# jweyn/DLWP-CS

Measured on AMD Instinct MI355X. Metric: cubed-sphere samples/sec (fwd+bwd), higher is better.
Workload: dtype bf16; 1 GPU; unet2 C48: x (32,6,48,48,14) per GPU, 14 out channels, base 32, MSE + Adam, fwd+bwd+update, bf16 activations + bf16 MFMA, fp32 master weights / gradients / Adam; global_batch=32, parallelism=dp1, hip_graphs=True

## Files before the change

dlwp-cs_amd/csrc/wgrad_batch.hip:

```cpp
#include <stdio.h>
#include <stdlib.h>
#include <string.h>
#include <vector>
#include "common.h"
#include "mfma_common.h"

namespace dlwpcs {
static const int g_wb_tags[] = {prof_register_tag("wgrad_batch_kernel"), prof_register_tag("wb_reduce_kernel"),
                                prof_register_tag("wb_reduce_kernel(apply)")};


constexpr int WB_MAX_LAYERS = DLWPCS_WGRAD_BATCH_MAX;
constexpr uint32_t WB_MAGIC = 0x57424c31u;

enum {
    WB_V_3_8_22 = 0,
    WB_V_3_8_21,
    WB_V_3_8_12,
    WB_V_3_8_11,
    WB_V_3_2_8,
    WB_V_3_2_16,
    WB_V_1_8_11,
    WB_V_1_8_D2,
    WB_V_F32_3,
    WB_V_F32_1,
    WB_V_F32_3_X2,
    WB_V_F32_3_H2,
    WB_V_F32_1_D2,
    WB_NVARIANTS
};

struct WbLayer {
    int32_t B, Nin, No, C0, C1, Cin, Cout, up0;
    int32_t halo, KS, W2, tile_rows_max, pix, nbands, pix_cap, variant;
    uint32_t magicW2, magicNo, magicN, magicB, magicNb;
    int32_t CT, NT, ncit, ncot, cin_logical, flip, want_bias, group_base, has_np, slot_floats, mask;
    float alpha, vmax;
    int32_t pad0, pad1;
};
static_assert(sizeof(WbLayer) == 144, "WbLayer layout");

struct WbSeg {
    int32_t layer, cls, cit, cot, t_first, t_last;
    uint32_t slot_off;
    int32_t bias;
};

struct WbGroup { uint32_t off, stride; int32_t count, pad; };

struct WbHeader {
    uint32_t magic, n_layers, n_segments, n_workers, n_groups, lds_bytes;
    uint32_t off_layers, off_segs, off_groups, total_bytes;
    uint64_t ws_floats;
    uint32_t red_first[WB_MAX_LAYERS + 1];
    uint32_t seg_start[257];
};

struct WbPtrs {
    const void *src0[WB_MAX_LAYERS], *src1[WB_MAX_LAYERS], *dz[WB_MAX_LAYERS], *y[WB_MAX_LAYERS];
    const int32_t *table[WB_MAX_LAYERS];
};
struct WbAdam {
    float *p, *g, *m, *v;
    const int32_t *state;
    const float *hyper;
    int32_t on;
    int32_t apply_only;
};
struct WbRedLayer { int32_t KS, Cin, Cout, want_bias, TC, TN, ncot, group_base, flip; };
struct WbRedPack { bf16_t *wf, *wb; float *bp; int32_t CGf, NTf, CGb, NTb, f32; };
struct WbPackArgs { WbRedPack l[WB_MAX_LAYERS]; };
struct WbRedPtrs {
    float *dw_eq[WB_MAX_LAYERS], *dw_pol[WB_MAX_LAYERS], *dw_np[WB_MAX_LAYERS];
    float *db_eq[WB_MAX_LAYERS], *db_pol[WB_MAX_LAYERS], *db_np[WB_MAX_LAYERS];
    uint32_t first[WB_MAX_LAYERS + 1];
    uint32_t live;
    uint32_t adam;
    uint32_t n_layers, off_groups;
    WbRedLayer lay[WB_MAX_LAYERS];
};

#ifndef DLWPCS_WB_SCHED
#define DLWPCS_WB_SCHED 1
#endif
template <int N> __device__ __forceinline__ void wb_sched_pairs() {
    if constexpr (N > 0) {
        __builtin_amdgcn_sched_group_barrier(0x008, 1, 0);
        __builtin_amdgcn_sched_group_barrier(0x100, 2, 0);
        wb_sched_pairs<N - 1>();
    }
}
#if DLWPCS_WB_SCHED == 1
#define WB_SCHED() do {                                                                   \
        __builtin_amdgcn_sched_group_barrier(0x100, 2, 0);       \
        wb_sched_pairs<TAPS>();                                                           \
    } while (0)
#else
#define WB_SCHED() do {                                                                   \
        __builtin_amdgcn_sched_group_barrier(0x100, 2 * TAPS + 2, 0);                     \
        __builtin_amdgcn_sched_group_barrier(0x008, TAPS, 0);                             \
    } while (0)
#endif

template <typename T> __device__ __forceinline__ T load_uniform(const T &g) {
    T out;
    const int *s = reinterpret_cast<const int *>(&g);
    int *d = reinterpret_cast<int *>(&out);
#pragma unroll
    for (int i = 0; i < (int)(sizeof(T) / 4); ++i) d[i] = __builtin_amdgcn_readfirstlane(s[i]);
    return out;
}

#define WB_SEG_ATTR __attribute__((noinline))
#ifndef DLWPCS_WB_PRODUCER_PRIO
#define DLWPCS_WB_PRODUCER_PRIO 0
#endif
#ifdef DLWPCS_WB_TL
constexpr int TL_WORKERS = 256, TL_MAX = 8;
#define WB_TL_DECL(kind_) \
    const bool tl_on = dbg != nullptr && (threadIdx.x & 255) == 0; \
    long long *tl_base = dbg + ((size_t)blockIdx.x * 2 + (kind_)) * TL_MAX; \
    long long tl_a[TL_MAX] = {0, 0, 0, 0, 0, 0, 0, 0}; \
    long long tl_prev = (long long)__builtin_amdgcn_s_memtime();
#define WB_TL(bucket_) do { const long long t_ = (long long)__builtin_amdgcn_s_memtime(); tl_a[bucket_] += t_ - tl_prev; tl_prev = t_; } while (0)
#define WB_TL_END() do { if (tl_on) { _Pragma("unroll") for (int q_ = 0; q_ < TL_MAX; ++q_) tl_base[q_] += tl_a[q_]; } } while (0)
#else
#define WB_TL_DECL(kind_)
#define WB_TL(tag_)
#define WB_TL_END()
#endif
template <int KS, int XV, int QX, int CT, int NT, int DV, bool MASK = false>
__device__ WB_SEG_ATTR void wb_segment(const WbLayer &Lg, const WbSeg &sgg, const void *src0, const void *src1,
                                           const void *dzp, const void *yp, const int32_t *table, float *ws, char *smem,
                                           long long *dbg) {
    const WbLayer L = load_uniform(Lg);
    const WbSeg sg = load_uniform(sgg);
    constexpr int QD = DV == 8 ? 4 : 8;
    constexpr int QDT = QD * NT;
    typedef typename VecT<bf16_t, DV>::type DVec;
    typedef typename VecT<bf16_t, XV>::type XVec;
    constexpr int TAPS = KS * KS;
    constexpr int PB = 64;
    constexpr int NCT = 256;
    constexpr int QXT = QX * CT;
    constexpr int IT_X = XV == 8 ? (CT == 2 ? 10 : 8) : 16;
    constexpr int CAP_PIX = (CT == 2 || NT == 2) ? 192 : 384;
    constexpr int IT_DY = CAP_PIX * QDT / NCT;
    constexpr int NPH = 4 / (CT * NT);
    constexpr int RSLOTS = TAPS - TAPS / NPH;
    constexpr int RED_FLOATS = 4 * RSLOTS * 1024;
    static_assert(CT * NT * NPH == 4, "four consumer waves");
    static_assert(CT == 1 || (XV == 8 && QX == 4), "two ci tiles per worker need full 16-B X vectors");
    static_assert(NCT % QXT == 0 && NCT % QDT == 0, "thread -> channel-vector maps must not depend on the item");

    const int pix_cap = L.pix_cap;
    constexpr int XCAP_PIX = (IT_X / CT) * NCT / QX;
    constexpr int plane_bytes = XCAP_PIX * PB;
    constexpr int x_bytes = CT * plane_bytes;
    constexpr int dzplane_bytes = CAP_PIX * PB;
    constexpr int buf_bytes = x_bytes + NT * dzplane_bytes;

    const int nfaces = sg.cls == 0 ? 4 : 1, fbase = sg.cls == 0 ? 0 : (sg.cls == 1 ? 4 : 5);
    const int n_my = sg.t_last - sg.t_first;
    const int face_pix = L.No * L.No;
    const int tid = threadIdx.x;
    (void)nfaces;

    struct Item { int b, f, combo, m0, npix, y0, nitems; };
    auto item_of = [&](int k) {
        Item it;
        const int t = sg.t_first + max(min(k, n_my - 1), 0);
        it.combo = L.magicB ? __umulhi((uint32_t)t, L.magicB) : t;
        it.b = t - it.combo * L.B;
        const int fl = L.magicNb ? __umulhi((uint32_t)it.combo, L.magicNb) : it.combo;
        const int band = it.combo - fl * L.nbands;
        it.f = fbase + fl;
        it.m0 = band * L.pix;
        it.npix = min(L.pix, face_pix - it.m0);
        it.y0 = __umulhi((uint32_t)it.m0, L.magicNo);
        const int ylast = __umulhi((uint32_t)(it.m0 + it.npix - 1), L.magicNo);
        it.nitems = (ylast - it.y0 + KS) * L.W2 * QXT;
        return it;
    };
    ws = reinterpret_cast<float *>(((uint64_t)(uint32_t)__builtin_amdgcn_readfirstlane((int)((uint64_t)ws >> 32)) << 32) |
                                   (uint32_t)__builtin_amdgcn_readfirstlane((int)(uint32_t)(uint64_t)ws));
    float *slot = ws + sg.slot_off;

    if (tid >= NCT) {
        const int ptid = tid - NCT;
        if (DLWPCS_WB_PRODUCER_PRIO) __builtin_amdgcn_s_setprio(DLWPCS_WB_PRODUCER_PRIO);
        WB_TL_DECL(0)
        const int qd = ptid % QDT;
        const int g0 = L.up0 ? (L.Nin >> 1) : L.Nin;
        const int M = L.Nin + KS - 1;
        const int co = sg.cot * 32 * NT + (qd / QD) * 32 + (qd % QD) * DV;
        const bool co_ok = co < L.Cout;
        const bool want_bias = sg.bias != 0;
        const uint32_t mthr1 = (uint32_t)L.pad0;
        float bsum[DV];
#pragma unroll
        for (int u = 0; u < DV; ++u) bsum[u] = 0.f;
        auto uni_ptr = [](const void *q) {
            return reinterpret_cast<const char *>(((uint64_t)(uint32_t)__builtin_amdgcn_readfirstlane((int)((uint64_t)q >> 32)) << 32) |
                                                  (uint32_t)__builtin_amdgcn_readfirstlane((int)(uint32_t)(uint64_t)q));
        };
        const char *const x0_u = uni_ptr(src0), *const x1_u = uni_ptr(src1);
        const char *const dz_u = uni_ptr(dzp), *const y_u = uni_ptr(yp);
        const int32_t *const table_u = reinterpret_cast<const int32_t *>(uni_ptr(table));
        const uint32_t s0_bytes = (uint32_t)((size_t)6 * g0 * g0 * L.C0 * 2), s1_bytes = (uint32_t)((size_t)6 * L.Nin * L.Nin * L.C1 * 2);
        constexpr int ITP = IT_X / CT;
        static_assert(IT_X % CT == 0 && NCT % QX == 0, "plane-major load map");
        const int qx = ptid % QX;
        struct Plane { int cs, stride; bool all0, up, ok, f0; };
        bool straddle = false;
        auto mkplane = [&](int pl) {
            Plane q;
            const int c_lo = sg.cit * 32 * CT + pl * 32, c_hi = min(c_lo + 32, L.Cin);
            const int cxp = c_lo + qx * XV;
            q.all0 = c_hi <= L.C0;
            straddle |= c_lo < L.C0 && c_hi > L.C0;
            q.ok = cxp < L.Cin;
            q.f0 = cxp < L.C0;
            q.cs = q.f0 ? cxp : cxp - L.C0;
            q.stride = q.f0 ? L.C0 : L.C1;
            q.up = q.f0 && L.up0;
            return q;
        };
        const Plane P0 = mkplane(0), P1 = mkplane(CT - 1);
        auto nit_plane = [&](const Item &it) { return it.nitems / CT; };
        uint32_t xoff[IT_X];
        int cur_combo = -1;
        const rsrc_t rt = make_rsrc(table_u, L.halo ? (uint32_t)(6 * M * M * 4) : 0u);
        auto rebuild = [&](const Item &it) {
            const int nitp = nit_plane(it);
            int tbl[ITP];
#pragma unroll
            for (int j = 0; j < ITP; ++j) {
                const int e = min(ptid + j * NCT, nitp - 1);
                const int pix = e / QX;
                const int ty = __umulhi((uint32_t)pix, L.magicW2);
                const int tx = pix - ty * L.W2;
                tbl[j] = (int)__builtin_amdgcn_raw_buffer_load_b32(rt, (uint32_t)(((it.f * M + it.y0 + ty) * M + tx) * 4), 0, 0);
            }
#pragma unroll
            for (int j = 0; j < ITP; ++j) {
                const int e = min(ptid + j * NCT, nitp - 1);
                const int pix = e / QX;
                const int ty = __umulhi((uint32_t)pix, L.magicW2);
                const int tx = pix - ty * L.W2;
                const int iy = it.y0 + ty;
                const int ii = L.halo ? tbl[j] : (it.f * L.Nin + iy) * L.Nin + tx;
                const int r = __umulhi((uint32_t)ii, L.magicN);
                const int pix_up = (r >> 1) * g0 + ((ii - r * L.Nin) >> 1);
                {
                    const int spix = P0.up ? pix_up : ii;
// ... 14 lines not shown
            DVec dv[IT_DY], yv[MASK ? IT_DY : 1];
        };
        auto bld = [](rsrc_t r, uint32_t off, auto &dst) __attribute__((always_inline)) {
            typedef std::remove_reference_t<decltype(dst)> V;
#ifdef DLWPCS_WB_ABL_P
            if (DLWPCS_WB_ABL_P & 2) { memset(&dst, 0, sizeof(V)); asm volatile("" : "+v"(*reinterpret_cast<uint32_t *>(&dst))); return; }
#endif
            if constexpr (sizeof(V) == 16) {
                const u32x4 q = __builtin_amdgcn_raw_buffer_load_b128(r, off, 0, 0);
                dst = make_uint4(q.x, q.y, q.z, q.w);
            } else {
                dst = __builtin_amdgcn_raw_buffer_load_b32(r, off, 0, 0);
            }
        };
        auto issue = [&](const Item &it, Stage &st, bool live) {
            if (live && it.combo != cur_combo) rebuild(it);
            const rsrc_t r0 = make_rsrc(x0_u + (size_t)it.b * s0_bytes, live ? s0_bytes : 0u);
            const rsrc_t r1 = make_rsrc(x1_u ? x1_u + (size_t)it.b * s1_bytes : nullptr, live ? s1_bytes : 0u);
            if (!straddle) {
                const rsrc_t rp0 = make_rsrc(P0.all0 ? x0_u + (size_t)it.b * s0_bytes : (x1_u ? x1_u + (size_t)it.b * s1_bytes : nullptr),
                                             live ? (P0.all0 ? s0_bytes : s1_bytes) : 0u);
                const rsrc_t rp1 = make_rsrc(P1.all0 ? x0_u + (size_t)it.b * s0_bytes : (x1_u ? x1_u + (size_t)it.b * s1_bytes : nullptr),
                                             live ? (P1.all0 ? s0_bytes : s1_bytes) : 0u);
#pragma unroll
                for (int i = 0; i < IT_X; ++i) {
                    if (i % CT == 0) bld(rp0, xoff[i], st.xv[i]);
                    else bld(rp1, xoff[i], st.xv[i]);
                }
            } else {
#pragma unroll
                for (int i = 0; i < IT_X; ++i) {
                    XVec a, b;
                    const bool f0 = i % CT == 0 ? P0.f0 : P1.f0;
                    bld(r0, f0 ? xoff[i] : 0xffffffffu, a);
                    bld(r1, f0 ? 0xffffffffu : xoff[i], b);
                    st.xv[i] = a | b;
                }
            }
            const size_t rowbase = (((size_t)it.b * 6 + it.f) * face_pix + it.m0) * L.Cout * 2;
            const uint32_t dbytes = live ? (uint32_t)(it.npix * L.Cout * 2) : 0u;
            const rsrc_t rd = make_rsrc(dz_u + rowbase, dbytes);
#pragma unroll
            for (int i = 0; i < IT_DY; ++i) bld(rd, doff[i], st.dv[i]);
            if constexpr (MASK) {
                const rsrc_t ry = make_rsrc(y_u + rowbase, dbytes);
#pragma unroll
                for (int i = 0; i < IT_DY; ++i) bld(ry, doff[i], st.yv[i]);
            }
        };
        auto commit = [&](const Item &it, int k, Stage &st) {
            char *buf = smem + (k & 1) * buf_bytes;
            WB_TL(0);
#ifdef DLWPCS_WB_TL
            asm volatile("s_waitcnt vmcnt(%0)" :: "n"(IT_X + IT_DY + (MASK ? IT_DY : 0)) : "memory");
            WB_TL(1);
#endif
            char *const xbase = buf + (ptid / QX) * PB + qx * (XV * 2);
#pragma unroll
            for (int i = 0; i < IT_X; ++i) {
#ifdef DLWPCS_WB_ABL_P
                if (DLWPCS_WB_ABL_P & 1) { asm volatile("" :: "v"(*reinterpret_cast<uint32_t *>(&st.xv[i]))); continue; }
#endif
                *reinterpret_cast<XVec *>(xbase + (i % CT) * plane_bytes + (i / CT) * (NCT / QX) * PB) = st.xv[i];
            }
            char *const dbase = buf + x_bytes + (qd / QD) * dzplane_bytes + (ptid / QDT) * PB + (qd % QD) * (DV * 2);
#pragma unroll
            for (int i = 0; i < IT_DY; ++i) {
                if constexpr (MASK) {
                    if constexpr (DV == 8) vmask_pk(st.dv[i], st.yv[i], L.alpha, mthr1);
                    else vmask(st.dv[i], st.yv[i], L.alpha, L.vmax);
                }
                const DVec v = st.dv[i];
#ifdef DLWPCS_WB_ABL_P
                if (DLWPCS_WB_ABL_P & 1) { asm volatile("" :: "v"(*reinterpret_cast<const uint32_t *>(&v))); }
                else
#endif
                *reinterpret_cast<DVec *>(dbase + i * (NCT / QDT) * PB) = v;
#ifdef DLWPCS_WB_ABL_P
                if (DLWPCS_WB_ABL_P & 4) continue;
#endif
                if (want_bias) {
                    if constexpr (DV == 8) {
                        bsum[0] += bf_lo(v.x); bsum[1] += bf_hi(v.x); bsum[2] += bf_lo(v.y); bsum[3] += bf_hi(v.y);
                        bsum[4] += bf_lo(v.z); bsum[5] += bf_hi(v.z); bsum[6] += bf_lo(v.w); bsum[7] += bf_hi(v.w);
                    } else {
                        bsum[0] += bf_lo(v); bsum[1] += bf_hi(v);
                    }
                }
            }
            asm volatile("s_waitcnt lgkmcnt(0)" ::: "memory");
            WB_TL(2);
            __builtin_amdgcn_s_barrier();
            WB_TL(3);
        };
        {
            Stage A, B;
            Item i0 = item_of(0), i1 = item_of(1);
            issue(i0, A, true);
            issue(i1, B, 1 < n_my);
            const int npair = n_my >> 1;
            for (int pr = 0; pr < npair; ++pr) {
                const int k = 2 * pr;
                commit(i0, k, A);
                i0 = item_of(k + 2);
                issue(i0, A, k + 2 < n_my);
                commit(i1, k + 1, B);
                i1 = item_of(k + 3);
                issue(i1, B, k + 3 < n_my);
            }
            if (n_my & 1) commit(i0, n_my - 1, A);
        }
        __syncthreads();
        float *red = reinterpret_cast<float *>(smem) + RED_FLOATS;
        if (want_bias) {
#pragma unroll
            for (int u = 0; u < DV; ++u) red[ptid * DV + u] = bsum[u];
        }
        __syncthreads();
        if (want_bias && ptid < 32 * NT) {
            float sum = 0.f;
            const int cc = ptid & 31, pl = ptid >> 5;
            if (cc < QD * DV) {
                const int q = pl * QD + cc / DV;
#pragma unroll 4
                for (int ph = 0; ph < NCT / QDT; ++ph) sum += red[(ph * QDT + q) * DV + (cc % DV)];
            }
            slot[TAPS * (32 * CT) * (32 * NT) + ptid] = sum;
        }
        __syncthreads();
        WB_TL(4);
        WB_TL_END();
        return;
    }

    const int lane = tid & 63, wave = tid >> 6;
    const int half = lane >> 5, l31 = lane & 31;
    const int li = lane & 15;
    WB_TL_DECL(1)
    const int choff = ((((lane >> 4) & 1) * 16) + (li & 3) * 4) * 2;
    const int prow = li >> 2;
    f32x16 acc[TAPS];
#pragma unroll
    for (int t = 0; t < TAPS; ++t)
#pragma unroll
        for (int r = 0; r < 16; ++r) acc[t][r] = 0.f;
    const int nslab = pix_cap / 16;
    const int S = (((nslab + NPH - 1) / NPH) + 1) & ~1;
    const int wave_u = __builtin_amdgcn_readfirstlane(wave);
    const int ct = wave_u % CT, nt = (wave_u / CT) % NT, ph = wave_u / (CT * NT);
    constexpr int DSTEP = 16 * NPH;
    const int stq = (int)__umulhi((uint32_t)DSTEP, L.magicNo), str = DSTEP - stq * L.No;
    const int stepA = (stq * L.W2 + str) * PB, wrapA = (L.W2 - L.No) * PB, rowB = L.W2 * PB;
    const int mlane = 16 * ph + 8 * half + prow;
    for (int k = 0; k < n_my; ++k) {
        WB_TL(1);
        __syncthreads();
        WB_TL(0);
        const int buf0 = (k & 1) * buf_bytes;
        const Item it = item_of(k);
        const int x0 = it.m0 - it.y0 * L.No;
        int xa[2], ox[2];
#pragma unroll
        for (int jj = 0; jj < 2; ++jj) {
            const int g = x0 + mlane + 4 * jj;
            const int oy = __umulhi((uint32_t)g, L.magicNo);
            ox[jj] = g - oy * L.No;
            xa[jj] = buf0 + ct * plane_bytes + (oy * L.W2 + ox[jj]) * PB + choff;
        }
        int da = buf0 + x_bytes + nt * dzplane_bytes + mlane * PB + choff;
        auto frag = [&](int si, uint4 (&a)[TAPS], uint4 &bq) {
            const int s = ph + NPH * si;
            const char *pd = smem + da + (s < nslab ? 0 : (1 << 23));
            const uint2 b0 = lds_tr16(pd), b1 = lds_tr16(pd + 4 * PB);
            bq = make_uint4(b0.x, b0.y, b1.x, b1.y);
#pragma unroll
            for (int ky = 0; ky < KS; ++ky) {
                const char *p0 = smem + xa[0] + ky * rowB, *p1 = smem + xa[1] + ky * rowB;
#pragma unroll
                for (int kx = 0; kx < KS; ++kx) {
#ifdef DLWPCS_WB_ABL_DS
                    if (DLWPCS_WB_ABL_DS == 1 && (ky | kx)) { a[ky * KS + kx] = a[0]; continue; }
                    if (DLWPCS_WB_ABL_DS == 3 && kx) { a[ky * KS + kx] = a[ky * KS]; continue; }
#endif
                    const uint2 a0 = lds_tr16(p0 + kx * PB), a1 = lds_tr16(p1 + kx * PB);
                    a[ky * KS + kx] = make_uint4(a0.x, a0.y, a1.x, a1.y);
                }
            }
            const bool nl = s + NPH < nslab;
            const int sr = nl ? str : 0, sa = nl ? stepA : 0;
#pragma unroll
            for (int jj = 0; jj < 2; ++jj) {
                const int o = ox[jj] + sr;
                const bool w = o >= L.No;
                ox[jj] = w ? o - L.No : o;
                xa[jj] += sa + (w ? wrapA : 0);
            }
            da += DSTEP * PB;
        };
        uint4 fa[2][TAPS], fb[2];
        frag(0, fa[0], fb[0]);
#ifdef DLWPCS_WB_TL
        asm volatile("s_waitcnt lgkmcnt(0)" ::: "memory");
        WB_TL(3);
#endif
        for (int si = 0; si < S; si += 2) {
            frag(si + 1, fa[1], fb[1]);
#pragma unroll
            for (int tap = 0; tap < TAPS; ++tap) frag_mma<bf16_t>(acc[tap], fb[0], fa[0][tap]);
            WB_SCHED();
            frag(si + 2, fa[0], fb[0]);
#pragma unroll
            for (int tap = 0; tap < TAPS; ++tap) frag_mma<bf16_t>(acc[tap], fb[1], fa[1][tap]);
            WB_SCHED();
        }
    }
    WB_TL(1);
    __syncthreads();
    float4 *red4 = reinterpret_cast<float4 *>(smem);
    const int wgrp = ct * NT + nt;
    auto slot_of = [](int t, int p) { int c = 0; for (int u = 0; u < t; ++u) c += (u % NPH != p) ? 1 : 0; return c; };
    if constexpr (NPH > 1) {
#pragma unroll
        for (int t = 0; t < TAPS; ++t) {
            if (ph != t % NPH) {
                float4 *dst = red4 + (size_t)((wgrp * NPH + ph) * RSLOTS + slot_of(t, ph)) * 256 + lane;
#pragma unroll
                for (int q = 0; q < 4; ++q)
                    dst[q * 64] = make_float4(acc[t][4 * q], acc[t][4 * q + 1], acc[t][4 * q + 2], acc[t][4 * q + 3]);
            }
        }
    }
    __syncthreads();
    const rsrc_t pr = make_rsrc(slot, (uint32_t)(TAPS * (32 * CT) * (32 * NT) * 4));
#pragma unroll
    for (int t = 0; t < TAPS; ++t) {
        if (ph == t % NPH) {
            f32x16 v[NPH];
#pragma unroll
            for (int p = 0; p < NPH; ++p) {
                if (p == t % NPH) { v[p] = acc[t]; continue; }
                if constexpr (NPH > 1) {
                    const float4 *src = red4 + (size_t)((wgrp * NPH + p) * RSLOTS + slot_of(t, p)) * 256 + lane;
#pragma unroll
                    for (int q = 0; q < 4; ++q) {
                        const float4 f = src[q * 64];
                        v[p][4 * q] = f.x; v[p][4 * q + 1] = f.y; v[p][4 * q + 2] = f.z; v[p][4 * q + 3] = f.w;
                    }
                }
            }
            const uint32_t row0 = (uint32_t)(((t * (32 * CT) + ct * 32 + l31) * (32 * NT) + nt * 32 + 4 * half) * 4);
#pragma unroll
            for (int q = 0; q < 4; ++q) {
                float sum[4];
#pragma unroll
                for (int u = 0; u < 4; ++u) {
                    const int r = 4 * q + u;
                    if (NPH == 4) sum[u] = (v[0][r] + v[1][r]) + (v[2][r] + v[3][r]);
                    else if (NPH == 2) sum[u] = v[0][r] + v[1][r];
                    else sum[u] = v[0][r];
                }
                bst128(make_uint4(__float_as_uint(sum[0]), __float_as_uint(sum[1]), __float_as_uint(sum[2]), __float_as_uint(sum[3])), pr,
                       row0 + (uint32_t)(8 * q * 4));
            }
        }
    }
    __syncthreads();
    WB_TL(2);
    WB_TL_END();
}

#ifndef DLWPCS_WB_F32_SCHED
#define DLWPCS_WB_F32_SCHED 2
#endif
#if DLWPCS_WB_F32_SCHED == 1
#define WB_F32_SCHED() do {                                                                                  \
        _Pragma("unroll") for (int t_ = 0; t_ < TAPS; ++t_) {                                                 \
            __builtin_amdgcn_sched_group_barrier(0x008, 1, 0);                                  \
            __builtin_amdgcn_sched_group_barrier(0x100, 1, 0);             \
            __builtin_amdgcn_sched_group_barrier(0x002, 2, 0);       \
        }                                                                                                     \
        __builtin_amdgcn_sched_group_barrier(0x100, 1, 0);                                                    \
    } while (0)
#elif DLWPCS_WB_F32_SCHED == 2
#define WB_F32_G(nread) do {                                                                                 \
        __builtin_amdgcn_sched_group_barrier(0x008, 1, 0);                                                    \
        if (nread) __builtin_amdgcn_sched_group_barrier(0x100, nread, 0);                                     \
        __builtin_amdgcn_sched_group_barrier(0x002, 2, 0);                                                    \
    } while (0)
#define WB_F32_SCHED() do {                                                                                  \
        if constexpr (TAPS == 9) {                                                                            \
            WB_F32_G(2); WB_F32_G(2); WB_F32_G(2); WB_F32_G(2); WB_F32_G(2);                                  \
            WB_F32_G(0); WB_F32_G(0); WB_F32_G(0); WB_F32_G(0);                                               \
        } else {                                                                                              \
            WB_F32_G(2);                                                                                      \
        }                                                                                                     \
    } while (0)
#else
#define WB_F32_SCHED() do {                                                                                  \
        __builtin_amdgcn_sched_group_barrier(0x100, TAPS + 1, 0);                                             \
        __builtin_amdgcn_sched_group_barrier(0x008, TAPS, 0);                                                 \
    } while (0)
#endif
template <int KS, bool MASK, bool X2 = false, bool D2 = false>
__device__ __attribute__((noinline)) void wb_segment_f32(const WbLayer &Lg, const WbSeg &sgg, const void *src0, const void *src1,
                                                       const void *dzp, const void *yp, const int32_t *table, float *ws, char *smem_raw) {
    const WbLayer L = load_uniform(Lg);
// ... 451 lines not shown
            *reinterpret_cast<VT *>(A.p + ai) = pv; *reinterpret_cast<VT *>(A.m + ai) = mv; *reinterpret_cast<VT *>(A.v + ai) = vv;
        }
    } else {
#pragma unroll
        for (int k = 0; k < VEC; ++k) {
            dst[k] = out[k];
            if (A.on) { A.p[ai + k] = pv[k]; A.m[ai + k] = mv[k]; A.v[ai + k] = vv[k]; }
        }
    }
}

__global__ void __launch_bounds__(256) wb_reduce_kernel(const char *__restrict__ plan, const WbRedPtrs R, const float *__restrict__ ws,
                                                        const WbAdam A, const dlwpcs_loss_tail tail, uint32_t red_blocks,
                                                        const WbPackArgs PK) {
    if (blockIdx.x >= red_blocks) {
        loss_stage2_body(tail.partial, tail.loss_out, tail.nblocks, tail.inv_n, tail.weight, tail.overwrite);
    } else if (threadIdx.x < WB_RED_THREADS) {
        const WbGroup *groups = reinterpret_cast<const WbGroup *>(plan + R.off_groups);
        const uint32_t b = blockIdx.x;
        int l = 0;
#pragma unroll
        for (int k = 1; k < WB_MAX_LAYERS; ++k) l += (k < (int)R.n_layers && b >= R.first[k]) ? 1 : 0;
        if ((R.live >> l) & 1u) {
            const WbRedLayer L = R.lay[l];
            WbAdam Al = A;
            if (!((R.adam >> l) & 1u)) Al.on = 0;
            const int blk = (int)(b - R.first[l]);
            const bool al = ((((uintptr_t)R.dw_eq[l] | (uintptr_t)R.dw_pol[l] | (uintptr_t)R.dw_np[l] | (uintptr_t)R.db_eq[l] |
                               (uintptr_t)R.db_pol[l] | (uintptr_t)R.db_np[l]) & 15) == 0);
            if (L.Cout % 4 == 0 && al)
                wb_reduce_body<4, true>(L, groups, ws, R.dw_eq[l], R.dw_pol[l], R.dw_np[l], R.db_eq[l], R.db_pol[l], R.db_np[l], blk, Al, PK.l[l]);
            else if (L.Cout % 4 == 0)
                wb_reduce_body<4, false>(L, groups, ws, R.dw_eq[l], R.dw_pol[l], R.dw_np[l], R.db_eq[l], R.db_pol[l], R.db_np[l], blk, Al, PK.l[l]);
            else
                wb_reduce_body<1, true>(L, groups, ws, R.dw_eq[l], R.dw_pol[l], R.dw_np[l], R.db_eq[l], R.db_pol[l], R.db_np[l], blk, Al, PK.l[l]);
        }
    }
    if (A.apply_only && (threadIdx.x < WB_RED_THREADS || blockIdx.x >= red_blocks)) {
        __syncthreads();
        if (threadIdx.x == 0) {
            int32_t *st = const_cast<int32_t *>(A.state);
            const int done = atomicAdd(st + 1, 1);
            if (done == (int)gridDim.x - 1) { st[1] = 0; st[0] += 1; }
        }
    }
}

static inline int wb_out_size(const dlwpcs_conv_desc *d) { return d->halo ? d->N : d->N - d->ksize + 1; }

static int wb_variant(const dlwpcs_conv_desc *d, int &CT, int &NT, int &cap_tile_px, int &cap_pix) {
    CT = NT = 1;
    if (d->dtype == DLWPCS_F32) {
        if (d->B < 1 || (d->ksize != 1 && d->ksize != 3) || (d->halo && d->ksize != 3) || (d->up0 && (d->N % 2))) return -1;
        if (!d->halo && d->N < d->ksize) return -1;
        if ((long)d->N * d->N >= (1l << 16)) return -1;
        if ((long)6 * d->N * d->N * (d->C0 > d->C1 ? d->C0 : d->C1) >= (1l << 31) || (long)6 * d->N * d->N * d->Cout >= (1l << 31)) return -1;
        cap_tile_px = 448; cap_pix = 192;
        if (d->C0 % 2 || d->C1 % 2 || d->Cout % 2 || (d->C1 > 0 && d->C0 % 4)) return -1;
        const bool x2 = d->C0 % 4 || d->C1 % 4, d2 = d->Cout % 4 != 0;
        if (d->ksize == 1) return x2 ? -1 : (d2 ? WB_V_F32_1_D2 : WB_V_F32_1);
        return x2 ? (d2 ? WB_V_F32_3_H2 : WB_V_F32_3_X2) : (d2 ? WB_V_F32_3_H2 : WB_V_F32_3);
    }
    if (d->dtype != DLWPCS_BF16 || d->B < 1 || (d->ksize != 1 && d->ksize != 3)) return -1;
    if (d->halo && d->ksize != 3) return -1;
    if (d->up0 && (d->N % 2)) return -1;
    if (!d->halo && d->N < d->ksize) return -1;
    if ((long)d->N * d->N >= (1l << 16)) return -1;
    if ((long)6 * d->N * d->N * (d->C0 > d->C1 ? d->C0 : d->C1) >= (1l << 31) || (long)6 * d->N * d->N * d->Cout >= (1l << 31))
        return -1;
    const int Cin = d->C0 + d->C1;
    const bool xv8 = d->C0 % 8 == 0 && d->C1 % 8 == 0;
    if (d->ksize == 3) {
        if (d->Cout % 8 != 0) return -1;
        if (xv8) {
            CT = Cin % 64 == 0 ? 2 : 1;
            NT = d->Cout % 64 == 0 ? 2 : 1;
            cap_tile_px = CT == 2 ? 320 : 512;
            cap_pix = (CT == 2 || NT == 2) ? 192 : 384;
            return CT == 2 ? (NT == 2 ? WB_V_3_8_22 : WB_V_3_8_21) : (NT == 2 ? WB_V_3_8_12 : WB_V_3_8_11);
        }
        if (d->C0 % 2 || d->C1 % 2 || Cin > 32) return -1;
        cap_pix = 384;
        if (Cin <= 16) { cap_tile_px = 512; return WB_V_3_2_8; }
        cap_tile_px = 256;
        return WB_V_3_2_16;
    }
    if (!xv8 || d->c0_valid != 0) return -1;
    if (Cin > 32) return -1;
    cap_tile_px = 512; cap_pix = 384;
    if (d->Cout % 8 == 0) return d->Cout <= 32 ? WB_V_1_8_11 : -1;
    if (d->Cout % 2 == 0 && d->Cout <= 16) return WB_V_1_8_D2;
    return -1;
}

struct WbGeom {
    WbLayer L;
    size_t lds;
    double cost_item[2];
};

static inline int wb_cin_logical(const dlwpcs_conv_desc *d) { return (d->c0_valid > 0 ? d->c0_valid : d->C0) + d->C1; }

static int wb_geometry(const dlwpcs_conv_desc *d, bool want_bias, bool has_np, bool mask, WbGeom &G) {
    int CT, NT, cap_tile_px, cap_pix;
    const int variant = wb_variant(d, CT, NT, cap_tile_px, cap_pix);
    if (variant < 0) return fail(DLWPCS_E_UNSUPPORTED, "wgrad_batch: layer (N=%d C0=%d C1=%d Cout=%d k=%d dtype=%d) has no batched kernel",
                                 d->N, d->C0, d->C1, d->Cout, d->ksize, d->dtype);
    const int KS = d->ksize, No = wb_out_size(d), face_pix = No * No, W2 = No + KS - 1;
    int CAP = cap_pix;
    auto pix_of = [&](int cap) { int p = cap; if (No <= cap) p = (cap / No) * No; if (p > face_pix) p = face_pix; return p; };
    while (CAP > 16 && (long)(tile_rows_for(pix_of(CAP), No) + KS - 1) * W2 > cap_tile_px) CAP -= (CAP > 96 ? 96 : 16);
    const int pix = pix_of(CAP);
    const int rows = tile_rows_for(pix, No) + KS - 1;
    if ((long)rows * W2 > cap_tile_px || pix < 1)
        return fail(DLWPCS_E_UNSUPPORTED, "wgrad_batch: a row of face size %d exceeds the producers' register capacity", No);
    WbLayer &L = G.L;
    memset(&L, 0, sizeof(L));
    L.B = d->B; L.Nin = d->N; L.No = No; L.C0 = d->C0; L.C1 = d->C1; L.Cin = d->C0 + d->C1; L.Cout = d->Cout; L.up0 = d->up0;
    L.halo = d->halo; L.KS = KS; L.W2 = W2; L.tile_rows_max = rows; L.pix = pix; L.nbands = ceil_div(face_pix, pix);
    const bool f32 = variant >= WB_V_F32_3;
    L.pix_cap = f32 ? (pix + 1) & ~1 : (pix + 15) & ~15; L.variant = variant;
    if ((long)d->B * 4 * L.nbands >= (1l << 16))
        return fail(DLWPCS_E_UNSUPPORTED, "wgrad_batch: %ld work items per face class exceed the 16-bit item arithmetic", (long)d->B * 4 * L.nbands);
    L.magicW2 = div_magic(W2); L.magicNo = div_magic(No); L.magicN = div_magic(d->N);
    L.magicB = d->B > 1 ? div_magic(d->B) : 0; L.magicNb = L.nbands > 1 ? div_magic(L.nbands) : 0;
    L.CT = CT; L.NT = NT;
    L.ncit = ceil_div(L.Cin, 32 * CT); L.ncot = ceil_div(d->Cout, 32 * NT);
    L.cin_logical = wb_cin_logical(d); L.flip = d->flip_north_pole ? 1 : 0; L.want_bias = want_bias ? 1 : 0;
    L.has_np = has_np ? 1 : 0;
    if (mask) {
        if (KS != 3) return fail(DLWPCS_E_UNSUPPORTED, "wgrad_batch: act' on load is built for the 3x3 kernels (pass a pre-masked dz)");
        if (d->act != DLWPCS_ACT_LEAKY_CLIP || !(d->alpha >= 0.f) || !(d->vmax >= 0.f))
            return fail(DLWPCS_E_INVALID, "wgrad_batch: item with y needs act = LEAKY_CLIP with negative_slope >= 0 and max_value >= 0");
        L.mask = 1; L.alpha = d->alpha; L.vmax = mask_vmax_for(d->dtype, d->vmax); L.pad0 = f32 ? 0 : (int32_t)bf16_mask_threshold(d->vmax);
    }
    const int TAPS = KS * KS;
    L.slot_floats = (int)align_up((size_t)TAPS * 32 * CT * 32 * NT + 32 * NT, 64);
    if (f32) {
        const size_t buf = ((size_t)rows * W2 + L.pix_cap) * 128;
        const size_t need = (size_t)(TAPS >= 3 ? 3 : 1) * 4 * 4096 + 4096;
        G.lds = 2 * buf > need ? 2 * buf : need;
        if (G.lds > 160 * 1024) return fail(DLWPCS_E_UNSUPPORTED, "wgrad_batch: LDS tile of %zu bytes exceeds 160 KiB", G.lds);
        const double cm[4] = {73.0, 4300.0, 6500.0, 7.5};
        const int nsteps = L.pix_cap / 2, S = (ceil_div(nsteps, 4) + 1) & ~1;
        const double cost = (double)S * TAPS * cm[0] + (KS == 1 ? cm[2] : cm[1]) + (mask ? cm[3] * pix : 0.0);
        G.cost_item[0] = G.cost_item[1] = cost;
        return DLWPCS_OK;
    }
    const size_t buf = (size_t)CT * cap_tile_px * 64 + (size_t)NT * cap_pix * 64;
    const int nph = 4 / (CT * NT), rslots = TAPS - TAPS / nph;
    const size_t need = ((size_t)4 * rslots * 1024 + 2048) * 4;
    G.lds = 2 * buf > need ? 2 * buf : need;
    if (G.lds > 160 * 1024) return fail(DLWPCS_E_UNSUPPORTED, "wgrad_batch: LDS tile of %zu bytes exceeds 160 KiB", G.lds);
    double fix = 3300.0, bpc = 35.0, slab3 = 570.0, slab1 = 260.0, ld4 = 45.0, cfix = 2000.0;
#ifdef DLWPCS_WB_TUNE_ENV
    if (const char *e = getenv("DLWPCS_WB_COST")) sscanf(e, "%lf,%lf,%lf,%lf,%lf,%lf", &fix, &bpc, &slab3, &slab1, &ld4, &cfix);
#endif
    const int nslab = L.pix_cap / 16;
    const int S = ((ceil_div(nslab, nph)) + 1) & ~1;
    const double mma = (double)S * (KS == 3 ? slab3 : slab1) + cfix;
    const bool x4 = variant == WB_V_3_2_8 || variant == WB_V_3_2_16, d4 = variant == WB_V_1_8_D2;
    for (int last = 0; last < 2; ++last) {
        int cin_grp = 32 * CT;
        if (last) { cin_grp = L.Cin - (L.ncit - 1) * 32 * CT; }
        const double xbytes = (double)rows * W2 * cin_grp * 2.0;
        const double dbytes = (double)pix * (d->Cout < 32 * NT ? d->Cout : 32 * NT) * 2.0 * (mask ? 2.0 : 1.0);
        double ld = fix + (xbytes + dbytes) / bpc;
        if (x4) ld += ld4 * ((double)rows * W2 * (variant == WB_V_3_2_8 ? 8 : 16) / 256.0);
        if (x4 && d->C1 > 0 && d->C0 % 32 != 0) ld = 4.0 * ld - 3.0 * fix;
        if (d4) ld += ld4 * ((double)pix * 8 / 256.0);
        if (mask) ld += 190.0 * ((double)pix * 4 * NT / 256.0);
        G.cost_item[last] = ld > mma ? ld : mma;
    }
    return DLWPCS_OK;
}

static double wb_seg_overhead() {
#ifdef DLWPCS_WB_TUNE_ENV
    if (const char *e = getenv("DLWPCS_WB_SEG")) return atof(e);
#endif
    return 20000.0;
}

struct WbPlanOut {
    WbHeader H;
    std::vector<WbLayer> layers;
    std::vector<WbSeg> segs;
    std::vector<WbGroup> groups;
};

static int wb_build(const dlwpcs_wgrad_item *items, int n, int n_workers, WbPlanOut &P) {
    if (n < 1 || n > WB_MAX_LAYERS) return fail(DLWPCS_E_INVALID, "wgrad_batch: %d items (1..%d)", n, WB_MAX_LAYERS);
    if (n_workers < 1 || n_workers > 256) return fail(DLWPCS_E_INVALID, "wgrad_batch: %d workers", n_workers);
    std::vector<WbGeom> G(n);
    size_t lds = 0;
    struct Grp { int layer, cit, cot, cls; long items; double cost_item; };
    std::vector<Grp> grps;
    double total = 0;
    int group_base = 0;
    uint32_t red_blocks = 0;
    memset(&P.H, 0, sizeof(P.H));
    for (int l = 0; l < n; ++l) {
        const dlwpcs_wgrad_item &it = items[l];
        const bool want_bias = it.db_eq || it.db_pol || it.db_np;
        int rc = wb_geometry(&it.d, want_bias, it.dw_np != nullptr, it.y != nullptr, G[l]);
        if (rc) return rc;
        if ((it.db_np != nullptr) != (it.dw_np != nullptr) && it.db_eq)
            return fail(DLWPCS_E_INVALID, "wgrad_batch: item %d: dw_np / db_np must match", l);
        WbLayer &L = G[l].L;
        L.group_base = group_base;
        group_base += L.ncit * L.ncot * 3;
        if (G[l].lds > lds) lds = G[l].lds;
        for (int cit = 0; cit < L.ncit; ++cit)
            for (int cot = 0; cot < L.ncot; ++cot)
                for (int cls = 0; cls < 3; ++cls) {
                    Grp g{l, cit, cot, cls, (long)L.B * (cls == 0 ? 4 : 1) * L.nbands, G[l].cost_item[cit == L.ncit - 1 ? 1 : 0]};
                    grps.push_back(g);
                    total += g.items * g.cost_item;
                }
        const int nout = L.KS * L.KS * L.cin_logical * L.Cout + (want_bias ? L.Cout : 0);
        P.H.red_first[l] = red_blocks;
        red_blocks += (uint32_t)ceil_div(L.Cout % 4 == 0 ? nout / 4 : nout, WB_RED_OUT);
    }
    for (int l = n; l <= WB_MAX_LAYERS; ++l) P.H.red_first[l] = red_blocks;
    const double seg_ovh = wb_seg_overhead();
    std::vector<uint32_t> seg_start(257, 0);
    auto pack = [&](double target, bool emit) -> bool {
        if (emit) P.segs.clear();
        int w = 0;
        double acc = 0;
        uint32_t nseg = 0;
        if (emit) seg_start[0] = 0;
        for (size_t gi = 0; gi < grps.size(); ++gi) {
            const Grp &g = grps[gi];
            long done = 0;
            while (done < g.items) {
                long take = (long)((target - acc - seg_ovh) / g.cost_item);
                if (take < 1) {
                    if (acc > 0) {
                        if (++w >= n_workers) return false;
                        if (emit) seg_start[w] = nseg;
                        acc = 0;
                        continue;
                    }
                    take = 1;
                }
                if (take > g.items - done) take = g.items - done;
                if (emit) {
                    WbSeg s{};
                    s.layer = g.layer; s.cls = g.cls; s.cit = g.cit; s.cot = g.cot;
                    s.t_first = (int)done; s.t_last = (int)(done + take);
                    s.bias = (G[g.layer].L.want_bias && g.cit == 0) ? 1 : 0;
                    P.segs.push_back(s);
                }
                ++nseg;
                acc += seg_ovh + take * g.cost_item;
                done += take;
            }
        }
        if (emit) for (int k = w + 1; k <= 256; ++k) seg_start[k] = nseg;
        return true;
    };
    double lo = total / n_workers, hi = total + (double)grps.size() * seg_ovh + 1.0;
    for (int it = 0; it < 40 && hi - lo > 1.0; ++it) {
        const double mid = 0.5 * (lo + hi);
        if (pack(mid, false)) hi = mid; else lo = mid;
    }
    if (!pack(hi, true)) return fail(DLWPCS_E_INVALID, "wgrad_batch: internal: the work list does not fit %d workers", n_workers);
    P.groups.assign((size_t)group_base, WbGroup{0, 0, 0, 0});
    uint64_t off = 0;
    for (size_t si = 0; si < P.segs.size(); ++si) {
        WbSeg &s = P.segs[si];
        const WbLayer &L = G[s.layer].L;
        WbGroup &g = P.groups[(size_t)L.group_base + (s.cit * L.ncot + s.cot) * 3 + s.cls];
        if (g.count == 0) { g.off = (uint32_t)off; g.stride = (uint32_t)L.slot_floats; }
        s.slot_off = (uint32_t)off;
        g.count += 1;
        off += (uint64_t)L.slot_floats;
        if (off >= (1ull << 32)) return fail(DLWPCS_E_UNSUPPORTED, "wgrad_batch: partial sums exceed 16 GiB");
    }
    P.layers.resize(n);
    for (int l = 0; l < n; ++l) P.layers[l] = G[l].L;
    WbHeader &H = P.H;
    H.magic = WB_MAGIC; H.n_layers = (uint32_t)n; H.n_segments = (uint32_t)P.segs.size(); H.n_workers = (uint32_t)n_workers;
    H.n_groups = (uint32_t)group_base; H.lds_bytes = (uint32_t)lds;
    H.off_layers = (uint32_t)align_up(sizeof(WbHeader), 256);
    H.off_segs = (uint32_t)align_up(H.off_layers + sizeof(WbLayer) * n, 256);
    H.off_groups = (uint32_t)align_up(H.off_segs + sizeof(WbSeg) * P.segs.size(), 256);
    H.total_bytes = (uint32_t)align_up(H.off_groups + sizeof(WbGroup) * P.groups.size(), 256);
    H.ws_floats = off;
    memcpy(H.seg_start, seg_start.data(), sizeof(H.seg_start));
    return DLWPCS_OK;
}

static int wb_workers() { return 256; }
#ifdef DLWPCS_WB_TL
static long long *g_tl_last = nullptr;
#endif

static size_t wb_plan_bound(int n_groups, int n_layers, int n_workers) {
    return align_up(sizeof(WbHeader), 256) + align_up(sizeof(WbLayer) * n_layers, 256) +
           align_up(sizeof(WbSeg) * (size_t)(n_groups + n_workers + 8), 256) + align_up(sizeof(WbGroup) * (size_t)n_groups, 256) + 256;
}

}

using namespace dlwpcs;

extern "C" int dlwpcs_wgrad_batch_supported(const dlwpcs_conv_desc *d) {
    if (!d) return 0;
    int CT, NT, a, b;
    if (wb_variant(d, CT, NT, a, b) < 0) return 0;
    WbGeom G;
// ... 227 lines not shown
```

Before: 47800 samples/s.

## Add row-walk path for 3x3 weight-gradient kernel reusing input rows across slabs

Adds a specialised loop for 3x3 weight-gradient tiles whose output width is a multiple of 16 and whose tile covers whole rows. Each wave walks down 16-pixel column strips row by row and keeps three input rows in registers in a rotating buffer, so each new output row needs only one new input row from LDS instead of reloading all taps. The loads use the ds_read_tr16 transpose instruction and a dedicated MFMA/LDS interleave schedule. The cost model gains a matching slab cost and drops the even-slab rounding for this path, which changes scheduling; the risks are higher register pressure and load imbalance from splitting strips across phases.

```diff
diff --git a/dlwp-cs_amd/csrc/wgrad_batch.hip b/dlwp-cs_amd/csrc/wgrad_batch.hip
--- a/dlwp-cs_amd/csrc/wgrad_batch.hip
+++ b/dlwp-cs_amd/csrc/wgrad_batch.hip
@@ -101,6 +101,16 @@
         __builtin_amdgcn_sched_group_barrier(0x008, TAPS, 0);                             \
     } while (0)
 #endif
+
+#define WB_SCHED_ROW() do {                                                               \
+        wb_sched_pairs<4>();                                                              \
+        __builtin_amdgcn_sched_group_barrier(0x008, 5, 0);                                \
+    } while (0)
+
+__device__ __forceinline__ uint2 lds_tr16_at(uint32_t a) {
+    const s16x4 v = __builtin_amdgcn_ds_read_tr16_b64_v4i16((__attribute__((address_space(3))) s16x4 *)(uintptr_t)a);
+    return __builtin_bit_cast(uint2, v);
+}
 
 template <typename T> __device__ __forceinline__ T load_uniform(const T &g) {
     T out;
@@ -421,6 +431,86 @@
     const int stq = (int)__umulhi((uint32_t)DSTEP, L.magicNo), str = DSTEP - stq * L.No;
     const int stepA = (stq * L.W2 + str) * PB, wrapA = (L.W2 - L.No) * PB, rowB = L.W2 * PB;
     const int mlane = 16 * ph + 8 * half + prow;
+    struct RwRun { int c, r, n, left; };
+    bool roww = false;
+    int rw_rows = 0, rw_cnt = 0;
+    RwRun rw0 = {0, 0, 0, 0};
+    if constexpr (KS == 3) {
+        rw_rows = (int)__umulhi((uint32_t)L.pix, L.magicNo);
+        roww = (L.No & 15) == 0 && rw_rows * L.No == L.pix;
+        if (roww) {
+            const int T = rw_rows * (L.No >> 4);
+            const int q0 = (ph * T) / NPH;
+            rw_cnt = ((ph + 1) * T) / NPH - q0;
+            rw0.c = q0 / rw_rows;
+            rw0.r = q0 - rw0.c * rw_rows;
+            rw0.n = min(rw_rows - rw0.r, rw_cnt);
+            rw0.left = rw_cnt - rw0.n;
+        }
+    }
+    if (roww) {
+        if constexpr (KS == 3) {
+            const int drow = L.No * PB;
+            const uint32_t rw_lds = (uint32_t)(uintptr_t)(__attribute__((address_space(3))) char *)smem;
+            auto ldrow = [&](uint4 (&row)[3], uint32_t a) __attribute__((always_inline)) {
+#pragma unroll
+                for (int kx = 0; kx < 3; ++kx) {
+                    const uint2 a0 = lds_tr16_at(a + kx * PB), a1 = lds_tr16_at(a + (kx + 4) * PB);
+                    row[kx] = make_uint4(a0.x, a0.y, a1.x, a1.y);
+                }
+            };
+            auto lddz = [&](uint4 &bq, uint32_t a) __attribute__((always_inline)) {
+                const uint2 b0 = lds_tr16_at(a), b1 = lds_tr16_at(a + 4 * PB);
+                bq = make_uint4(b0.x, b0.y, b1.x, b1.y);
+            };
+            for (int k = 0; k < n_my; ++k) {
+                WB_TL(1);
+                __syncthreads();
+                WB_TL(0);
+                if (rw_cnt == 0) continue;
+                const int buf0 = (k & 1) * buf_bytes;
+                const uint32_t xb = rw_lds + buf0 + ct * plane_bytes + (8 * half + prow) * PB + choff;
+                uint32_t da = rw_lds + buf0 + x_bytes + nt * dzplane_bytes + (8 * half + prow) * PB + choff + (rw0.r * L.No + 16 * rw0.c) * PB;
+                RwRun run = rw0;
+                for (;;) {
+                    uint32_t xa = xb + run.c * (16 * PB) + run.r * rowB;
+                    uint4 S0[3], S1[3], S2[3], S3[3], fa, fbn;
+                    ldrow(S0, xa);
+                    ldrow(S1, xa + rowB);
+                    ldrow(S2, xa + 2 * rowB);
+                    lddz(fa, da);
+                    xa += (run.n > 1 ? 3 : 2) * rowB;
+                    auto slab = [&](int q, const uint4 &f, uint4 &fnext, const uint4 (&k0)[3], const uint4 (&k1)[3], const uint4 (&k2)[3],
+                                    uint4 (&rnext)[3]) __attribute__((always_inline)) {
+                        da += q + 1 < run.n ? drow : 0;
+                        lddz(fnext, da);
+                        ldrow(rnext, xa);
+                        xa += q + 2 < run.n ? rowB : 0;
+#pragma unroll
+                        for (int kx = 0; kx < 3; ++kx) frag_mma<bf16_t>(acc[kx], f, k0[kx]);
+#pragma unroll
+                        for (int kx = 0; kx < 3; ++kx) frag_mma<bf16_t>(acc[3 + kx], f, k1[kx]);
+#pragma unroll
+                        for (int kx = 0; kx < 3; ++kx) frag_mma<bf16_t>(acc[6 + kx], f, k2[kx]);
+                        WB_SCHED_ROW();
+                    };
+                    for (int i = 0; i < run.n; i += 4) {
+                        slab(i, fa, fbn, S0, S1, S2, S3);
+                        if (i + 1 < run.n) {
+                            slab(i + 1, fbn, fa, S1, S2, S3, S0);
+                            if (i + 2 < run.n) {
+                                slab(i + 2, fa, fbn, S2, S3, S0, S1);
+                                if (i + 3 < run.n) slab(i + 3, fbn, fa, S3, S0, S1, S2);
+                            }
+                        }
+                    }
+                    if (run.left == 0) break;
+                    da += 16 * PB - (run.r + run.n - 1) * drow;
+                    run.c += 1; run.r = 0; run.n = min(rw_rows, run.left); run.left -= run.n;
+                }
+            }
+        }
+    } else
     for (int k = 0; k < n_my; ++k) {
         WB_TL(1);
         __syncthreads();
@@ -1178,13 +1268,15 @@
     const size_t need = ((size_t)4 * rslots * 1024 + 2048) * 4;
     G.lds = 2 * buf > need ? 2 * buf : need;
     if (G.lds > 160 * 1024) return fail(DLWPCS_E_UNSUPPORTED, "wgrad_batch: LDS tile of %zu bytes exceeds 160 KiB", G.lds);
-    double fix = 3300.0, bpc = 35.0, slab3 = 570.0, slab1 = 260.0, ld4 = 45.0, cfix = 2000.0;
+    double fix = 3300.0, bpc = 35.0, slab3 = 570.0, slab1 = 260.0, ld4 = 45.0, cfix = 2000.0, slab3r = 570.0;
 #ifdef DLWPCS_WB_TUNE_ENV
-    if (const char *e = getenv("DLWPCS_WB_COST")) sscanf(e, "%lf,%lf,%lf,%lf,%lf,%lf", &fix, &bpc, &slab3, &slab1, &ld4, &cfix);
+    if (const char *e = getenv("DLWPCS_WB_COST"))
+        if (sscanf(e, "%lf,%lf,%lf,%lf,%lf,%lf,%lf", &fix, &bpc, &slab3, &slab1, &ld4, &cfix, &slab3r) < 7) slab3r = slab3;
 #endif
     const int nslab = L.pix_cap / 16;
-    const int S = ((ceil_div(nslab, nph)) + 1) & ~1;
-    const double mma = (double)S * (KS == 3 ? slab3 : slab1) + cfix;
+    const bool roww = KS == 3 && No % 16 == 0 && pix % No == 0;
+    const int S = roww ? ceil_div(nslab, nph) : ((ceil_div(nslab, nph)) + 1) & ~1;
+    const double mma = (double)S * (KS == 3 ? (roww ? slab3r : slab3) : slab1) + cfix;
     const bool x4 = variant == WB_V_3_2_8 || variant == WB_V_3_2_16, d4 = variant == WB_V_1_8_D2;
     for (int last = 0; last < 2; ++last) {
         int cin_grp = 32 * CT;
```

Result: no change. 47570 samples/s, median of 2 (-0.5%).
